# alex-petrenko/sample-factory

Hardware: NVIDIA H100
Metric: env-steps/sec (sampler+learner) at 4096 envs (higher is better)
Workload: dtype f32 (3-pass tf32 hi/lo operand split on wgmma, fp32 accumulate)

## Files before the change

### sample_factory_b200/csrc/rollout_fused.cu

```cuda
#include <cuda.h>

#include <cstdlib>

#include "common.cuh"
#include "gemm.h"
#include "heads_tail.cuh"
#include "tc_ptx.cuh"
#include "wgmma_tile.cuh"

namespace sfb {

constexpr int RF_THREADS = 384;
constexpr int RF_HEAD_AP = 9;
constexpr int RF_MAX_DIM = 128;
constexpr int RF_PRODUCER_REGS = 40;
constexpr int RF_CONSUMER_REGS = 232;

__host__ __device__ __forceinline__ bool rf_wide(int H2) { return H2 >= 256; }
__host__ __device__ __forceinline__ int rf_bm(int H2) { return rf_wide(H2) ? 64 : 128; }
__host__ __device__ __forceinline__ int rf_bn(int H2) { return rf_wide(H2) ? 256 : 128; }

template <bool F16>
struct RfSmem {
    static constexpr int STAGES = 2;
    static constexpr int KBK = F16 ? 64 : TBK;
    __host__ __device__ static constexpr int slot(int bm, int bn) { return F16 ? (bm + bn) * 256 : (bm + 3 * bn) * 128; }
    __host__ __device__ static constexpr int a_bytes(int bm) { return bm * KBK * 4; }
    __host__ __device__ static constexpr int b_hi(int bm, int bn) { return F16 ? bm * 256 : (bm + bn) * 128; }
    __host__ __device__ static constexpr int stage_tx(int bm, int bn) { return (bm + bn) * KBK * 4; }
    static constexpr int OFF_PART = STAGES * slot(64, 256) + 64 * 256;
    static constexpr int OFF_B1 = OFF_PART + (F16 ? 256 * kHeadPartPad * 4 : 0);
    static constexpr int OFF_B2 = OFF_B1 + (F16 ? 256 * 4 : 0);
    static constexpr int OFF_HW = OFF_B2 + (F16 ? 256 * 4 : 0);
    static constexpr int OFF_HB = OFF_HW + (F16 ? RF_HEAD_AP * 256 * 4 : 0);
    static constexpr int OFF_BARS = OFF_HB + (F16 ? 16 * 4 : 0);
    static constexpr int OFF_CSTAT = OFF_BARS + 64;
    static constexpr int TOTAL = OFF_CSTAT + 2 * RF_MAX_DIM * 4 + 1024 ;
    static_assert(2 * STAGES * 8 <= 64 && TOTAL + 64 <= 227 * 1024, "shared memory");
    static_assert(STAGES * slot(128, 128) + 128 * 256 <= OFF_PART, "the 128 x 128 layout fits below the partials");
};


struct RolloutArgs {
    int64_t N; int T, K1, H1, H2;
    const float* b1; const float* b2; const float* wv; const float* wa; int A; const float* bv; const float* ba;
    float* h1; float* part; float* x_norm;
    float* values; int64_t values_rs; float* logits; int64_t logits_rs; float* actions; int64_t actions_rs;
    int32_t* env_actions; float* log_prob; int64_t lp_rs; float* pv_out; int64_t pv_rs; const float* pv_scalar;
    const float* noise; uint64_t seed; int64_t* sampler_step;
    const float* tape; int64_t tape_len; int64_t env_off; int term_period, trunc_period; int64_t* env_step;
    float* env_obs; float* env_rew; uint8_t* env_term; uint8_t* env_trunc;
    float reward_scale, reward_clip; int32_t policy_id; float* t_rew; uint8_t* t_done; uint8_t* t_to; int32_t* t_pid; int64_t stride;
    float* ep_ret; int32_t* ep_len; float* ep_min; float* ep_max; int32_t len_inc; double* stats; float* fin_ret; int32_t* fin_len;
    float* traj_obs; int64_t traj_obs_rs; const float* rnn; int rnn_dim; float* traj_rnn; int64_t traj_rnn_rs;
    const double* mean; const double* var; float sub, inv_scale; int do_sub, do_scale; float eps, clip;
    unsigned int* ticket;
    unsigned long long* trace;
    const float* bound_x; const float* bound_h1;
};

__device__ __forceinline__ void cluster_arrive() { asm volatile("barrier.cluster.arrive.release.aligned;" ::: "memory"); }
__device__ __forceinline__ void cluster_wait() { asm volatile("barrier.cluster.wait.acquire.aligned;" ::: "memory"); }
__device__ __forceinline__ void cluster_sync_all() {
    cluster_arrive();
    cluster_wait();
}
__device__ __forceinline__ void fence_proxy_async_all() { asm volatile("fence.proxy.async.global;" ::: "memory"); }
__device__ __forceinline__ unsigned long long rf_now() {
    unsigned long long t;
    asm volatile("mov.u64 %0, %%globaltimer;" : "=l"(t));
    return t;
}
__device__ __forceinline__ uint32_t smid() {
    uint32_t r;
    asm volatile("mov.u32 %0, %%smid;" : "=r"(r));
    return r;
}
__device__ __forceinline__ uint32_t mapa_shared(uint32_t addr, uint32_t rank) {
    uint32_t r;
    asm volatile("mapa.shared::cluster.u32 %0, %1, %2;" : "=r"(r) : "r"(addr), "r"(rank));
    return r;
}
__device__ __forceinline__ void st_cluster_f4(uint32_t addr, float4 v) {
    asm volatile("st.shared::cluster.v4.f32 [%0], {%1, %2, %3, %4};" ::"r"(addr), "f"(v.x), "f"(v.y), "f"(v.z), "f"(v.w)
                 : "memory");
}
__device__ __forceinline__ uint32_t cluster_ctarank() {
    uint32_t r;
    asm volatile("mov.u32 %0, %%cluster_ctarank;" : "=r"(r));
    return r;
}

template <bool F16>
__device__ __forceinline__ void rf_produce(const CUtensorMap* tmap_x, const CUtensorMap* tmap_w1, const CUtensorMap* tmap_h1,
                                           const CUtensorMap* tmap_w2, int T, int K1, int H1, int bm, int bn, int m0, int n0,
                                           uint8_t* smem, uint64_t* full, uint64_t* empty, bool leader) {
    using S = RfSmem<F16>;
    constexpr int KBK = S::KBK;
    const int slot_bytes = S::slot(bm, bn), b_off = S::a_bytes(bm);
    const uint32_t stage_tx = (uint32_t)S::stage_tx(bm, bn);
    const int n1 = K1 / KBK, n2 = H1 / KBK;
    uint32_t pu = 0;
    auto weight = [&](const CUtensorMap* tb, int kb) {
        const uint32_t s = pu % S::STAGES;
        mbar_wait(&empty[s], ((pu / S::STAGES) & 1) ^ 1);
        mbar_expect_tx(&full[s], stage_tx);
        uint8_t* dst = smem + s * slot_bytes + b_off;
        if (F16) tma_load_3d(dst, tb, &full[s], 64 * kb, n0, 0);
        else tma_load_2d(dst, tb, &full[s], TBK * kb, n0);
        ++pu;
    };
    auto activation = [&](uint32_t u, const CUtensorMap* ta, bool planes, int kb) {
        const uint32_t s = u % S::STAGES;
        if (planes) tma_load_3d(smem + s * slot_bytes, ta, &full[s], 64 * kb, m0, 0);
        else tma_load_2d(smem + s * slot_bytes, ta, &full[s], KBK * kb, m0);
    };
    const int pre2 = n2 < S::STAGES ? n2 : S::STAGES;
    int pre1 = 0;
    for (int t = 0; t < T; ++t) {
        if (leader) {
            fence_proxy_async_all();
            const uint32_t u1 = pu - pre1;
            for (int j = 0; j < n1; ++j) {
                if (j >= pre1) weight(tmap_w1, j);
                activation(u1 + j, tmap_x, false, j);
            }
        }
        __syncwarp();
        cluster_arrive();
        const uint32_t u2 = pu;
        if (leader)
            for (int j = 0; j < pre2; ++j) weight(tmap_w2, j);
        __syncwarp();
        cluster_wait();
        if (leader) {
            fence_proxy_async_all();
            for (int j = 0; j < n2; ++j) {
                if (j >= pre2) weight(tmap_w2, j);
                activation(u2 + j, tmap_h1, F16, j);
            }
        }
        __syncwarp();
        cluster_arrive();
        pre1 = t + 1 < T ? (n1 < S::STAGES ? n1 : S::STAGES) : 0;
        if (leader)
            for (int j = 0; j < pre1; ++j) weight(tmap_w1, j);
        __syncwarp();
        cluster_wait();
        cluster_sync_all();
    }
}

template <bool F16, bool SPLIT_A>
__device__ __forceinline__ void rf_tile(int nkb, bool wide, uint8_t* smem, uint64_t* full, uint64_t* empty, uint32_t& cu,
                                        float (&acc)[64], float (&cross)[64], int ct, int a_shift, unsigned long long* tr,
                                        int s_land, int s_split, int s_done) {
    using S = RfSmem<F16>;
    const int wg = ct >> 7, lt = ct & 127;
    const int bm = wide ? 64 : 128, bn = wide ? 256 : 128;
    const int slot_bytes = S::slot(bm, bn), b_hi = S::b_hi(bm, bn);
    const int a_row = wide ? 0 : 64 * wg, b_row = wide ? 128 * wg : 0;
    uint8_t* conv = smem + S::STAGES * slot_bytes;
#pragma unroll
    for (int i = 0; i < 64; ++i) acc[i] = cross[i] = 0.f;
    int held = -1;
    for (int kb = 0; kb < nkb; ++kb, ++cu) {
        const int s = (int)(cu % S::STAGES);
        uint8_t* slot = smem + s * slot_bytes;
        mbar_wait(&full[s], (cu / S::STAGES) & 1);
        if (tr && kb == nkb - 1) tr[s_land] = rf_now();
        const uint8_t* at = slot;
        if (SPLIT_A || !F16) {
            if (held >= 0) {
                wgmma_wait_all();
                mbar_arrive(&empty[held]);
                held = -1;
                if (wide) consumer_sync();
            }
            if constexpr (F16) {
                if (wide) split_tile_f16<false, 64, 256>(slot, conv, conv + 8192, ct, pow2f_int(a_shift));
                else split_tile_f16<false, 64>(slot + wg * 64 * 256, conv + wg * 8192, conv + 16384 + wg * 8192, lt,
                                               pow2f_int(a_shift));
            } else if (wide) {
                split_tile<false, true, 64, 256>(slot, conv, conv + 8192, ct);
                split_tile<false, true, 256, 256>(slot + 8192, slot + b_hi, slot + b_hi + 32768, ct);
            } else {
                split_tile<false, true, 64>(slot + wg * 64 * 128, conv + wg * 8192, conv + 16384 + wg * 8192, lt);
                split_tile<false, true>(slot + 16384, slot + b_hi, slot + b_hi + 16384, ct);
            }
            fence_proxy_async_smem();
            consumer_sync();
            if (tr && kb == nkb - 1) tr[s_split] = rf_now();
            at = conv;
        }
        const uint64_t da_hi = make_smem_desc(smem_u32(at + a_row * 128));
        const uint64_t da_lo = make_smem_desc(smem_u32(at + bm * 128 + a_row * 128));
        const uint64_t db_hi = make_smem_desc(smem_u32(slot + b_hi + b_row * 128));
        const uint64_t db_lo = make_smem_desc(smem_u32(slot + b_hi + bn * 128 + b_row * 128));
        wgmma_fence();
#pragma unroll
        for (int k = 0; k < TBK / WG_K; ++k) {
            const uint64_t o = (uint64_t)(2 * k);
            if constexpr (F16) {
                wgmma_m64n128k16_f16(acc, da_hi + o, db_hi + o, (kb | k) != 0);
                wgmma_m64n128k16_f16(cross, da_hi + o, db_lo + o, (kb | k) != 0);
                wgmma_m64n128k16_f16(cross, da_lo + o, db_hi + o, 1);
            } else {
                wgmma_m64n128k8_tf32(acc, da_hi + o, db_hi + o, (kb | k) != 0);
                wgmma_m64n128k8_tf32(cross, da_hi + o, db_lo + o, (kb | k) != 0);
                wgmma_m64n128k8_tf32(cross, da_lo + o, db_hi + o, 1);
            }
        }
        wgmma_commit();
        if (held >= 0) {
            wgmma_wait_1();
            mbar_arrive(&empty[held]);
        }
        held = s;
    }
    wgmma_wait_all();
    if (tr) tr[s_done] = rf_now();
    mbar_arrive(&empty[held]);
    if (F16) {
        const float out_scale = pow2f_int(-(a_shift + kF16WShift));
#pragma unroll
        for (int i = 0; i < 64; ++i) acc[i] = fmaf(cross[i], 1.f / 2048.f, acc[i]) * out_scale;
    } else {
#pragma unroll
        for (int i = 0; i < 64; ++i) acc[i] += cross[i];
    }
}

__device__ __forceinline__ void store_h1_split(const float (&acc)[64], int n0, int64_t row_base, int lane, uint16_t* hi,
                                               int64_t lo_off, int64_t M, int H1, const float* bias, int act, float scale) {
    float b[32];
    const float* bp = bias + 2 * (lane & 3);
#pragma unroll
    for (int c = 0; c < 16; ++c) {
        b[2 * c] = bp[8 * c];
        b[2 * c + 1] = bp[8 * c + 1];
    }
#pragma unroll
    for (int j = 0; j < 32; ++j) {
        const int64_t m = row_base + 8 * (j & 1);
        const int n = n0 + 8 * (j >> 1) + 2 * (lane & 3);
        if (m >= M) continue;
        const float v0 = act_fwd_fast(acc[2 * j] + b[j & ~1], act);
        const float v1 = act_fwd_fast(acc[2 * j + 1] + b[j | 1], act);
        uint32_t h, l;
        f16_split2(v0 * scale, v1 * scale, h, l);
        uint16_t* dst = hi + m * H1 + n;
        *reinterpret_cast<uint32_t*>(dst) = h;
        *reinterpret_cast<uint32_t*>(dst + lo_off) = l;
    }
}

template <int ACT>
__device__ __forceinline__ void rf_heads_tile(float (&acc)[64], int nl, int p0, int rb, int lane, const float* b2,
                                              const float* hw, int A, uint32_t part, int rpc) {
    constexpr int JP = 16;
    const int nq = nl + 2 * (lane & 3);
    float b[32];
#pragma unroll
    for (int c = 0; c < 16; ++c) {
        b[2 * c] = b2[nq + 8 * c];
        b[2 * c + 1] = b2[nq + 8 * c + 1];
    }
#pragma unroll
    for (int j = 0; j < 32; ++j) {
        acc[2 * j] = act_fwd_ct<ACT>(acc[2 * j] + b[j & ~1]);
        acc[2 * j + 1] = act_fwd_ct<ACT>(acc[2 * j + 1] + b[j | 1]);
    }
#pragma unroll
    for (int half = 0; half < 2; ++half) {
        float hp[2][kHeadAP];
#pragma unroll
        for (int a = 0; a < kHeadAP; ++a) {
            float s[2] = {0.f, 0.f};
            if (a <= A) {
                const float* w = hw + a * 256 + nq + 64 * half;
                float2 wv[JP / 2];
#pragma unroll
                for (int jj = 0; jj < JP / 2; ++jj) wv[jj] = *reinterpret_cast<const float2*>(w + 8 * jj);
#pragma unroll
                for (int jj = 0; jj < JP / 2; ++jj) {
#pragma unroll
                    for (int rs = 0; rs < 2; ++rs) {
                        const int j = JP * half + 2 * jj + rs;
                        s[rs] = fmaf(acc[2 * j], wv[jj].x, s[rs]);
                        s[rs] = fmaf(acc[2 * j + 1], wv[jj].y, s[rs]);
                    }
                }
            }
#pragma unroll
            for (int rs = 0; rs < 2; ++rs) {
                s[rs] += __shfl_xor_sync(0xffffffffu, s[rs], 1);
                s[rs] += __shfl_xor_sync(0xffffffffu, s[rs], 2);
                hp[rs][a] = s[rs];
            }
        }
        if ((lane & 3) == 0) {
#pragma unroll
            for (int rs = 0; rs < 2; ++rs) {
                const int r = rb + 8 * rs;
                const uint32_t dst =
                    mapa_shared(part + (uint32_t)(((p0 + half) * rpc + r % rpc) * kHeadPartPad * 4), (uint32_t)(r / rpc));
                st_cluster_f4(dst, make_float4(hp[rs][0], hp[rs][1], hp[rs][2], hp[rs][3]));
                st_cluster_f4(dst + 16, make_float4(hp[rs][4], hp[rs][5], hp[rs][6], hp[rs][7]));
                st_cluster_f4(dst + 32, make_float4(hp[rs][8], 0.f, 0.f, 0.f));
            }
        }
    }
}

template <int ACT, bool F16>
__global__ void __launch_bounds__(RF_THREADS, 1)
rollout_mlp2_tape_kernel(const __grid_constant__ CUtensorMap tmap_x, const __grid_constant__ CUtensorMap tmap_w1,
                         const __grid_constant__ CUtensorMap tmap_h1, const __grid_constant__ CUtensorMap tmap_w2,
                         const RolloutArgs a) {
    using S = RfSmem<F16>;
    constexpr int KBK = S::KBK;
    extern __shared__ uint8_t smem_raw[];
    uint8_t* smem = smem_align_1024(smem_raw);
    uint64_t* full = reinterpret_cast<uint64_t*>(smem + S::OFF_BARS);
    uint64_t* empty = full + S::STAGES;
    float* cstat = reinterpret_cast<float*>(smem + S::OFF_CSTAT);
    float* s_part = reinterpret_cast<float*>(smem + S::OFF_PART);
    float* s_b1 = reinterpret_cast<float*>(smem + S::OFF_B1);
    float* s_b2 = reinterpret_cast<float*>(smem + S::OFF_B2);
    float* s_hw = reinterpret_cast<float*>(smem + S::OFF_HW);
    float* s_hb = reinterpret_cast<float*>(smem + S::OFF_HB);

    __shared__ double s_stats[5];
    const int warp = threadIdx.x >> 5, lane = threadIdx.x & 31;
    if (threadIdx.x < 5) s_stats[threadIdx.x] = 0.0;
    const int cx = (int)cluster_ctarank();
    const int CX = gridDim.x;
    const bool wide = rf_wide(a.H2);
    const int BM = rf_bm(a.H2), BN = rf_bn(a.H2);
    const int n0 = cx * BN;
    const int64_t m0 = (int64_t)blockIdx.y * BM;
    const int P = a.H2 / 64;
    const bool do_rms = a.mean != nullptr;
    unsigned long long* cta_trace =
        a.trace ? a.trace + (int64_t)a.T * 16 + 4 * ((int64_t)blockIdx.y * gridDim.x + blockIdx.x) : nullptr;
    if (cta_trace && threadIdx.x == 0) {
        cta_trace[0] = smid();
        cta_trace[1] = rf_now();
    }

    if (threadIdx.x == 0) {
        asm volatile("prefetch.tensormap [%0];" ::"l"(&tmap_x) : "memory");
        asm volatile("prefetch.tensormap [%0];" ::"l"(&tmap_w1) : "memory");
        asm volatile("prefetch.tensormap [%0];" ::"l"(&tmap_h1) : "memory");
        asm volatile("prefetch.tensormap [%0];" ::"l"(&tmap_w2) : "memory");
        for (int s = 0; s < S::STAGES; ++s) {
            mbar_init(&full[s], 1);
            mbar_init(&empty[s], 256);
        }
        fence_barrier_init();
    }
    __syncthreads();
    pdl_wait();
    pdl_trigger();
    if (cta_trace && threadIdx.x == 0) cta_trace[2] = rf_now();
    if (do_rms)
        for (int c = threadIdx.x; c < a.K1; c += RF_THREADS) col_stats(a.mean, a.var, c, a.eps, cstat[c], cstat[a.K1 + c]);
    if (F16) {
        for (int i = threadIdx.x; i < BN; i += RF_THREADS) {
            s_b1[i] = a.b1[n0 + i];
            s_b2[i] = a.b2[n0 + i];
            s_hw[i] = a.wv[n0 + i];
            for (int r = 0; r < a.A; ++r) s_hw[(r + 1) * 256 + i] = a.wa[(int64_t)r * a.H2 + n0 + i];
        }
        if (threadIdx.x <= a.A) s_hb[threadIdx.x] = threadIdx.x == 0 ? a.bv[0] : a.ba[threadIdx.x - 1];
    }
    __syncthreads();
    const int64_t env_step0 = a.env_step[0];
    const uint64_t philox0 = a.sampler_step ? (uint64_t)*a.sampler_step : 0ull;

    if (warp < 4) {
        setmaxnreg_dec<RF_PRODUCER_REGS>();
        rf_produce<F16>(&tmap_x, &tmap_w1, &tmap_h1, &tmap_w2, a.T, a.K1, a.H1, BM, BN, (int)m0, n0, smem, full, empty,
                        threadIdx.x == 0);
    } else {
        setmaxnreg_inc<RF_CONSUMER_REGS>();
        const float pv = a.pv_scalar ? *a.pv_scalar : 0.f;
        const int shift_x = F16 ? f16_shift_for_bound(a.bound_x[0]) : 0;
        const int shift_h = F16 ? f16_shift_for_bound(a.bound_h1[0]) : 0;
        const bool tracer = a.trace != nullptr && blockIdx.x == 0 && blockIdx.y == 0 && threadIdx.x == 128;
#define RF_TRACE(slot) do { if (tracer) a.trace[(int64_t)t * 16 + (slot)] = rf_now(); } while (0)
        uint32_t cu = 0;
        const TcEpilogue epi_heads{1, ACT, a.b2, nullptr, 0, a.wv, a.wa, a.A, a.part};
        const TcEpilogue epi_h1{1, ACT, a.b1, nullptr, 0};
        const int ct = threadIdx.x - 128;
        const int64_t row_base = m0 + (wide ? 0 : (ct >> 7) * 64) + ((ct >> 5) & 3) * 16 + (lane >> 2);
        TileCoord tc;
        tc.m0 = m0; tc.n0 = n0 + (wide ? (ct >> 7) * 128 : 0); tc.k_begin = 0; tc.num_kb = 0; tc.z = 0;

        for (int t = 0; t < a.T; ++t) {
            RF_TRACE(0);
            unsigned long long* const tr = tracer ? a.trace + (int64_t)t * 16 : nullptr;
            {
                float acc[64], cross[64];
                rf_tile<F16, true>(a.K1 / KBK, wide, smem, full, empty, cu, acc, cross, ct, shift_x, tr, 1, 2, 5);
                if (F16)
                    store_h1_split(acc, tc.n0, row_base, lane, reinterpret_cast<uint16_t*>(a.h1), a.N * a.H1, a.N, a.H1,
                                   s_b1 + (tc.n0 - n0), ACT, pow2f_int(shift_h));
                else
                    store_tile(acc, tc, row_base, lane, a.h1, a.H1, a.N, a.H1, 1, epi_h1);
                RF_TRACE(6);
                fence_proxy_async_all();
                RF_TRACE(3);
            }
            cluster_sync_all();
            RF_TRACE(4);
            {
                float acc[64], cross[64];
                rf_tile<F16, !F16>(a.H1 / KBK, wide, smem, full, empty, cu, acc, cross, ct, shift_h, tr, 11, 14, 12);
                if (F16)
                    rf_heads_tile<ACT>(acc, tc.n0 - n0, tc.n0 / 64, (int)(row_base - m0), lane, s_b2, s_hw, a.A,
                                       smem_u32(s_part), BM / CX);
                else
                    heads_tile<ACT>(acc, tc, row_base, lane, nullptr, 0, a.N, a.H2, epi_heads);
                RF_TRACE(7);
            }
            cluster_sync_all();
            RF_TRACE(8);

            {
                const int g = lane & 7;
                const int grp = lane >> 3;
                const int act_idx = (g + 7) & 7;
                const bool has_logit = act_idx < a.A;
                const bool leader = g == 0;
                const bool last = (t + 1 == a.T);
                const int64_t step = env_step0 + t;
                const uint64_t offset = philox0 + (uint64_t)t;
                const float* src_step = a.tape + ((step + 1) % a.tape_len) * a.N * a.K1;
                const float* noise_t = a.noise ? a.noise + (int64_t)t * a.N * a.A : nullptr;
                const int rpc = BM / CX;
                const unsigned gmask = 0xffu << (grp * 8);
                for (int base = 0; base < rpc; base += 32) {
                    const int rr = base + (warp - 4) * 4 + grp;
                    const int64_t row = m0 + cx * rpc + rr;
                    const bool ok = rr < rpc && row < a.N;
                    float x = 0.f, val = 0.f;
                    float ob[RF_MAX_DIM / 8];
                    float er0 = 0.f, mn0 = 0.f, mx0 = 0.f;
                    int32_t el0 = 0;
                    const int cpl = a.K1 >> 3;
                    if (ok) {
                        if (F16) {
                            if (has_logit)
                                for (int p = 0; p < P; ++p) x += s_part[(p * rpc + rr) * kHeadPartPad + 1 + act_idx];
                            if (leader)
                                for (int p = 0; p < P; ++p) val += s_part[(p * rpc + rr) * kHeadPartPad];
                        } else {
                            if (has_logit)
                                for (int p = 0; p < P; ++p) x += a.part[((int64_t)p * a.N + row) * kHeadPartPad + 1 + act_idx];
                            if (leader)
                                for (int p = 0; p < P; ++p) val += a.part[((int64_t)p * a.N + row) * kHeadPartPad];
                        }
                        const float4* src4 = reinterpret_cast<const float4*>(src_step + row * a.K1 + g * cpl);
#pragma unroll
                        for (int q = 0; q < RF_MAX_DIM / 32; ++q)
                            if (4 * q < cpl) {
                                const float4 f4 = src4[q];
                                ob[4 * q] = f4.x; ob[4 * q + 1] = f4.y; ob[4 * q + 2] = f4.z; ob[4 * q + 3] = f4.w;
                            }
                        if (leader && a.ep_ret) { er0 = a.ep_ret[row]; el0 = a.ep_len[row]; mn0 = a.ep_min[row]; mx0 = a.ep_max[row]; }
                    }
                    if (tr && base == 0) tr[13] = tc_now_after(val);
                    x += has_logit ? (F16 ? s_hb[1 + act_idx] : a.ba[act_idx]) : 0.f;
                    val += F16 ? s_hb[0] : a.bv[0];
                    const float xl = has_logit ? x : -INFINITY;
                    float m = xl;
#pragma unroll
                    for (int o = 4; o > 0; o >>= 1) m = fmaxf(m, __shfl_xor_sync(0xffffffffu, m, o));
                    const float ex = has_logit ? expf(xl - m) : 0.f;
                    float ssum = ex;
#pragma unroll
                    for (int o = 4; o > 0; o >>= 1) ssum += __shfl_xor_sync(0xffffffffu, ssum, o);
                    const float pr = __fdiv_rn(ex, ssum);
                    const float logp = (xl - m) - logf(ssum);
                    float q = 1.f;
                    if (ok && has_logit) {
                        if (noise_t) q = noise_t[row * a.A + act_idx];
                        else {
                            curandStatePhilox4_32_10_t st;
                            curand_init(a.seed, (unsigned long long)(row * a.A + act_idx), offset, &st);
                            q = fmaxf(-logf(curand_uniform(&st)), 1.0e-30f);
                        }
                    }
                    float best = has_logit ? __fdiv_rn(pr, q) : -INFINITY;
                    int idx = has_logit ? act_idx : 0x7fffffff;
#pragma unroll
                    for (int o = 4; o > 0; o >>= 1) {
                        const float ob_ = __shfl_xor_sync(0xffffffffu, best, o);
                        const int oi = __shfl_xor_sync(0xffffffffu, idx, o);
                        if (ob_ > best || (ob_ == best && oi < idx)) { best = ob_; idx = oi; }
                    }
                    const float lp = __shfl_sync(0xffffffffu, logp, (grp << 3) | ((idx + 1) & 7));
                    if (tr && base == 0) tr[15] = tc_now_after(lp);
                    (void)gmask;
                    if (!ok) continue;
                    if (has_logit) a.logits[row * a.logits_rs + (int64_t)t * a.A + act_idx] = x;
                    const int64_t env = a.env_off + row;
                    const float r_raw = (float)idx / (float)a.A;
                    const bool tm = ((step * 7 + env * 13) % a.term_period) == 0;
                    const bool tr = (((step + env) % a.trunc_period) == 0) && !tm;
                    float* obs_next = a.traj_obs + row * a.traj_obs_rs + (int64_t)(t + 1) * a.K1 + g * cpl;
                    float* env_o = a.env_obs + row * a.K1 + g * cpl;
                    float* xn = a.x_norm + row * a.K1 + g * cpl;
#pragma unroll
                    for (int q4 = 0; q4 < RF_MAX_DIM / 32; ++q4)
                        if (4 * q4 < cpl) {
                            const float4 f4 = make_float4(ob[4 * q4], ob[4 * q4 + 1], ob[4 * q4 + 2], ob[4 * q4 + 3]);
                            reinterpret_cast<float4*>(env_o)[q4] = f4;
                            reinterpret_cast<float4*>(obs_next)[q4] = f4;
                            if (!last) {
                                const int c = g * cpl + 4 * q4;
                                float4 y;
                                y.x = norm_one(f4.x, a.sub, a.inv_scale, a.do_sub, a.do_scale, do_rms, do_rms ? cstat[c] : 0.f, do_rms ? cstat[a.K1 + c] : 1.f, a.clip);
                                y.y = norm_one(f4.y, a.sub, a.inv_scale, a.do_sub, a.do_scale, do_rms, do_rms ? cstat[c + 1] : 0.f, do_rms ? cstat[a.K1 + c + 1] : 1.f, a.clip);
                                y.z = norm_one(f4.z, a.sub, a.inv_scale, a.do_sub, a.do_scale, do_rms, do_rms ? cstat[c + 2] : 0.f, do_rms ? cstat[a.K1 + c + 2] : 1.f, a.clip);
                                y.w = norm_one(f4.w, a.sub, a.inv_scale, a.do_sub, a.do_scale, do_rms, do_rms ? cstat[c + 3] : 0.f, do_rms ? cstat[a.K1 + c + 3] : 1.f, a.clip);
                                reinterpret_cast<float4*>(xn)[q4] = y;
                            }
                        }
                    if (a.rnn)
                        for (int j = g; j < a.rnn_dim; j += 8)
                            a.traj_rnn[row * a.traj_rnn_rs + (int64_t)(t + 1) * a.rnn_dim + j] = a.rnn[row * a.rnn_dim + j];
                    if (leader) {
                        a.values[row * a.values_rs + t] = val;
                        a.actions[row * a.actions_rs + t] = (float)idx;
                        a.env_actions[row] = idx;
                        a.log_prob[row * a.lp_rs + t] = lp;
                        a.pv_out[row * a.pv_rs + t] = pv;
                        a.env_rew[row] = r_raw;
                        a.env_term[row] = tm;
                        a.env_trunc[row] = tr;
                        const bool done = tm || tr;
                        float r = __fmul_rn(r_raw, a.reward_scale);
                        r = clampf(r, -a.reward_clip, a.reward_clip);
                        a.t_rew[row * a.stride + t] = r;
                        a.t_done[row * a.stride + t] = done ? 1 : 0;
                        a.t_to[row * a.stride + t] = tr ? 1 : 0;
                        a.t_pid[row * a.stride + t] = a.policy_id;
                        if (a.ep_ret) {
                            float er = er0 + r_raw;
                            int32_t el = el0 + a.len_inc;
                            float mn = fminf(mn0, r_raw), mx = fmaxf(mx0, r_raw);
                            if (a.fin_ret) {
                                a.fin_ret[row * a.stride + t] = done ? er : __int_as_float(0x7fc00000);
                                a.fin_len[row * a.stride + t] = done ? el : -1;
                            }
                            if (done) {
                                if (a.stats) {
                                    atomicAdd(&s_stats[0], 1.0); atomicAdd(&s_stats[1], (double)er); atomicAdd(&s_stats[2], (double)el);
                                    atomicAdd(&s_stats[3], (double)mn); atomicAdd(&s_stats[4], (double)mx);
                                }
                                er = 0.f; el = 0; mn = INFINITY; mx = -INFINITY;
                            }
                            a.ep_ret[row] = er; a.ep_len[row] = el; a.ep_min[row] = mn; a.ep_max[row] = mx;
                        }
                    }
                }
                fence_proxy_async_all();
                RF_TRACE(9);
            }

            cluster_sync_all();
            RF_TRACE(10);
        }
#undef RF_TRACE
    }

    __syncthreads();
    if (threadIdx.x < 5 && a.stats && s_stats[0] > 0.0) atomicAdd(a.stats + threadIdx.x, s_stats[threadIdx.x]);
    if (threadIdx.x == 0) {
        if (cta_trace) cta_trace[3] = rf_now();
        __threadfence();
        if (atomicAdd(a.ticket, 1u) == gridDim.x * gridDim.y - 1u) {
            *a.ticket = 0u;
            a.env_step[0] = env_step0 + a.T;
            if (a.sampler_step) *a.sampler_step = (int64_t)philox0 + a.T;
        }
    }
}

template <int ACT, bool F16>
static int rollout_launch_config(int64_t N, int H2, cudaStream_t st, cudaLaunchConfig_t& cfg, cudaLaunchAttribute (&attr)[2]) {
    auto kern = rollout_mlp2_tape_kernel<ACT, F16>;
    static bool attr_set = false;
    if (!attr_set) {
        SFB_CUDA_OK(cudaFuncSetAttribute(kern, cudaFuncAttributeMaxDynamicSharedMemorySize, RfSmem<F16>::TOTAL));
        attr_set = true;
    }
    const int CX = H2 / rf_bn(H2);
    cfg = {};
    cfg.gridDim = dim3((unsigned)CX, (unsigned)ceil_div(N, rf_bm(H2)));
    cfg.blockDim = dim3(RF_THREADS);
    cfg.dynamicSmemBytes = RfSmem<F16>::TOTAL;
    cfg.stream = st;
    attr[0].id = cudaLaunchAttributeClusterDimension;
    attr[0].val.clusterDim.x = (unsigned)CX;
    attr[0].val.clusterDim.y = 1;
    attr[0].val.clusterDim.z = 1;
    attr[1].id = cudaLaunchAttributeProgrammaticStreamSerialization;
    attr[1].val.programmaticStreamSerializationAllowed = 1;
    cfg.attrs = attr;
    cfg.numAttrs = pdl_enabled() ? 2 : 1;
    return 0;
}

template <int ACT, bool F16>
static int launch_rollout(const CUtensorMap* tm, const RolloutArgs& a, cudaStream_t st) {
    cudaLaunchConfig_t cfg;
    cudaLaunchAttribute attr[2];
    const int rc = rollout_launch_config<ACT, F16>(a.N, a.H2, st, cfg, attr);
    if (rc) return rc;
    SFB_CUDA_OK(cudaLaunchKernelEx(&cfg, rollout_mlp2_tape_kernel<ACT, F16>, tm[0], tm[1], tm[2], tm[3], a));
    SFB_LAUNCH_OK();
    return 0;
}

template <int ACT, bool F16>
static int rollout_occupancy(int64_t N, int H2, int* needed, int* resident) {
    cudaLaunchConfig_t cfg;
    cudaLaunchAttribute attr[2];
    const int rc = rollout_launch_config<ACT, F16>(N, H2, 0, cfg, attr);
    if (rc) return rc;
    SFB_CUDA_OK(cudaOccupancyMaxActiveClusters(resident, rollout_mlp2_tape_kernel<ACT, F16>, &cfg));
    *needed = (int)(cfg.gridDim.x * cfg.gridDim.y / attr[0].val.clusterDim.x);
    return 0;
}

int tc_rollout_mlp2_supported(const float* W1, const float* W2, int K1, int H1, int H2, int A, int engine) {
    if (engine != SFB200_GEMM_TC_3XTF32 || !tc_init()) return 0;
    if (!(K1 == 32 || K1 == 64 || K1 == 96 || K1 == 128) || H1 != H2 || !(H2 == 128 || H2 == 256 || H2 == 512)) return 0;
    if (A < 1 || A + 1 > RF_HEAD_AP) return 0;
    if ((reinterpret_cast<uintptr_t>(W1) & 15u) || (reinterpret_cast<uintptr_t>(W2) & 15u)) return 0;
    return 2 * (H2 / 128);
}

static bool rollout_f16_enabled() {
    static int v = -1;
    if (v < 0) {
        const char* e = getenv("SFB200_TC_F16");
        v = (e && e[0] == '0') ? 0 : 1;
    }
    return v == 1;
}

#define SFB_RF_LAUNCH(F16v)                                                                  \
    switch (act) {                                                                           \
        case SFB200_ACT_ELU: return launch_rollout<SFB200_ACT_ELU, F16v>(tm, a, st);     \
        case SFB200_ACT_RELU: return launch_rollout<SFB200_ACT_RELU, F16v>(tm, a, st);   \
        case SFB200_ACT_TANH: return launch_rollout<SFB200_ACT_TANH, F16v>(tm, a, st);   \
        default: return launch_rollout<SFB200_ACT_NONE, F16v>(tm, a, st);                \
    }

static int g_rollout_form = -1;

int tc_rollout_mlp2_tape(const float* W1, const float* W2, int act, int engine, const RolloutArgs& a_in, cudaStream_t st) {
    if (!tc_rollout_mlp2_supported(W1, W2, a_in.K1, a_in.H1, a_in.H2, a_in.A, engine)) return SFB_TC_UNSUPPORTED;
    if ((reinterpret_cast<uintptr_t>(a_in.wv) & 7u) || (reinterpret_cast<uintptr_t>(a_in.wa) & 7u)) return SFB_TC_UNSUPPORTED;
    RolloutArgs a = a_in;
    const uint32_t BM = (uint32_t)rf_bm(a.H2), BN = (uint32_t)rf_bn(a.H2);
    if (rollout_f16_enabled() && a.K1 % 64 == 0 && a.H1 % 64 == 0) {
        const F16Twin t1 = f16_twin_lookup(W1, (int64_t)a.H1 * a.K1), t2 = f16_twin_lookup(W2, (int64_t)a.H2 * a.H1);
        const float* bx = operand_bound_lookup(a.x_norm, a.N * a.K1 * (int64_t)sizeof(float));
        const float* bh = operand_bound_lookup(a.h1, a.N * a.H1 * (int64_t)sizeof(float));
        if (t1.hi && t2.hi && bx && bh) {
            if (f16_check_enabled()) {
                int rc = f16_twins_check(W1, t1, a.H1, a.K1, false, st);
                if (!rc) rc = f16_twins_check(W2, t2, a.H2, a.H1, false, st);
                if (rc) return rc;
            }
            a.bound_x = bx;
            a.bound_h1 = bh;
            CUtensorMap tm[4];
            bool ok = make_tmap(&tm[0], a.x_norm, (uint64_t)a.K1, (uint64_t)a.N, (uint64_t)a.K1, 64, BM);
            ok = ok && make_tmap_f16_twins(&tm[1], t1.hi, t1.lo - t1.hi, (uint64_t)a.K1, (uint64_t)a.H1, BN);
            ok = ok && make_tmap_f16_twins(&tm[2], reinterpret_cast<const uint16_t*>(a.h1), a.N * a.H1, (uint64_t)a.H1,
                                           (uint64_t)a.N, BM);
            ok = ok && make_tmap_f16_twins(&tm[3], t2.hi, t2.lo - t2.hi, (uint64_t)a.H1, (uint64_t)a.H2, BN);
            if (ok) {
                g_rollout_form = 1;
                SFB_RF_LAUNCH(true)
            }
        }
    }
    a.bound_x = a.bound_h1 = nullptr;
    CUtensorMap tm[4];
    bool ok = make_tmap(&tm[0], a.x_norm, (uint64_t)a.K1, (uint64_t)a.N, (uint64_t)a.K1, TBK, BM);
    ok = ok && make_tmap(&tm[1], W1, (uint64_t)a.K1, (uint64_t)a.H1, (uint64_t)a.K1, TBK, BN);
    ok = ok && make_tmap(&tm[2], a.h1, (uint64_t)a.H1, (uint64_t)a.N, (uint64_t)a.H1, TBK, BM);
    ok = ok && make_tmap(&tm[3], W2, (uint64_t)a.H1, (uint64_t)a.H2, (uint64_t)a.H1, TBK, BN);
    if (!ok) return SFB_TC_UNSUPPORTED;
    g_rollout_form = 0;
    SFB_RF_LAUNCH(false)
}
#undef SFB_RF_LAUNCH

}

using namespace sfb;

extern "C" {

static unsigned long long* g_rollout_trace = nullptr;
int sfb200_rollout_set_trace(void* trace_dev) {
    g_rollout_trace = (unsigned long long*)trace_dev;
    return 0;
}

int sfb200_rollout_last_form(void) { return g_rollout_form; }

int sfb200_rollout_occupancy(int64_t n_envs, int K1, int H1, int H2, int A, int engine, int act, int* clusters_needed,
                             int* clusters_resident) {
    SFB_CHECK_ARG(n_envs > 0 && clusters_needed && clusters_resident, "rollout_occupancy: bad arguments");
    SFB_CHECK_ARG(tc_rollout_mlp2_supported(nullptr, nullptr, K1, H1, H2, A, engine),
                  "rollout_occupancy: model not covered (K1=%d H1=%d H2=%d A=%d engine=%d)", K1, H1, H2, A, engine);
    if (rollout_f16_enabled() && K1 % 64 == 0 && H1 % 64 == 0) {
        switch (act) {
            case SFB200_ACT_ELU: return rollout_occupancy<SFB200_ACT_ELU, true>(n_envs, H2, clusters_needed, clusters_resident);
            case SFB200_ACT_RELU: return rollout_occupancy<SFB200_ACT_RELU, true>(n_envs, H2, clusters_needed, clusters_resident);
            case SFB200_ACT_TANH: return rollout_occupancy<SFB200_ACT_TANH, true>(n_envs, H2, clusters_needed, clusters_resident);
            default: return rollout_occupancy<SFB200_ACT_NONE, true>(n_envs, H2, clusters_needed, clusters_resident);
        }
    }
    switch (act) {
        case SFB200_ACT_ELU: return rollout_occupancy<SFB200_ACT_ELU, false>(n_envs, H2, clusters_needed, clusters_resident);
        case SFB200_ACT_RELU: return rollout_occupancy<SFB200_ACT_RELU, false>(n_envs, H2, clusters_needed, clusters_resident);
        case SFB200_ACT_TANH: return rollout_occupancy<SFB200_ACT_TANH, false>(n_envs, H2, clusters_needed, clusters_resident);
        default: return rollout_occupancy<SFB200_ACT_NONE, false>(n_envs, H2, clusters_needed, clusters_resident);
    }
}

int sfb200_rollout_mlp2_partials(const float* W1, const float* W2, int K1, int H1, int H2, int A, int engine) {
    return tc_rollout_mlp2_supported(W1, W2, K1, H1, H2, A, engine);
}

int sfb200_rollout_mlp2_tape(int64_t n_envs, int T, int K1, const float* W1, const float* b1, int H1, const float* W2,
                             const float* b2, int H2, int act, int engine, const float* Wv, const float* bv, const float* Wa,
                             const float* ba, int A, float* h1_scratch, float* head_partials, float* x_norm,
                             float* values_0, int64_t values_stride, float* logits_0, int64_t logits_stride,
                             const float* noise, uint64_t philox_seed, int64_t* sampler_step, float* actions_0,
                             int64_t actions_stride, int32_t* env_actions, float* log_prob_0, int64_t log_prob_stride,
                             const float* policy_version_scalar, float* policy_version_0, int64_t pv_stride,
                             const float* tape, int64_t tape_len, int64_t env_index_offset, int term_period, int trunc_period,
                             int64_t* env_step_counter, float* env_obs, float* env_rew, uint8_t* env_terminated,
                             uint8_t* env_truncated, float reward_scale, float reward_clip, int32_t policy_id,
                             float* traj_rewards_0, uint8_t* traj_dones_0, uint8_t* traj_time_outs_0, int32_t* traj_policy_id_0,
                             int64_t traj_stride, float* ep_return, int32_t* ep_len, float* ep_min_raw, float* ep_max_raw,
                             int32_t len_increment, double* stats, float* fin_return_0, int32_t* fin_len_0, float* traj_obs_0,
                             int64_t traj_obs_stride, const float* rnn, int rnn_dim, float* traj_rnn_0, int64_t traj_rnn_stride,
                             const double* mean, const double* var, float sub_mean, float inv_scale, float eps, float clip,
                             void* stream) {
    SFB_CHECK_ARG(n_envs > 0 && T > 0 && W1 && b1 && W2 && b2 && Wv && bv && Wa && ba && h1_scratch && head_partials && x_norm,
                  "rollout_mlp2_tape: bad model arguments");
    SFB_CHECK_ARG(values_0 && logits_0 && actions_0 && env_actions && log_prob_0 && policy_version_0 && policy_version_scalar,
                  "rollout_mlp2_tape: bad heads arguments");
    SFB_CHECK_ARG(tape && tape_len > 0 && term_period > 0 && trunc_period > 0 && env_step_counter && env_obs && env_rew &&
                      env_terminated && env_truncated, "rollout_mlp2_tape: bad env arguments");
    SFB_CHECK_ARG(traj_rewards_0 && traj_dones_0 && traj_time_outs_0 && traj_policy_id_0 && traj_obs_0,
                  "rollout_mlp2_tape: bad trajectory arguments");
    SFB_CHECK_ARG((mean == nullptr) == (var == nullptr), "rollout_mlp2_tape: mean/var must both be set or both NULL");
    SFB_CHECK_ARG(K1 <= RF_MAX_DIM, "rollout_mlp2_tape: observation rows of up to %d floats", RF_MAX_DIM);
    SFB_CHECK_ARG((reinterpret_cast<uintptr_t>(h1_scratch) & 15u) == 0 && (reinterpret_cast<uintptr_t>(x_norm) & 15u) == 0 &&
                      (reinterpret_cast<uintptr_t>(head_partials) & 15u) == 0, "rollout_mlp2_tape: scratch buffers must be 16-byte aligned");
    const bool with_rnn = rnn && traj_rnn_0 && rnn_dim > 0;
    unsigned int* ticket = reinterpret_cast<unsigned int*>(env_step_counter + 1);
    const RolloutArgs a{n_envs, T, K1, H1, H2, b1, b2, Wv, Wa, A, bv, ba, h1_scratch, head_partials, x_norm,
                        values_0, values_stride, logits_0, logits_stride, actions_0, actions_stride, env_actions, log_prob_0,
                        log_prob_stride, policy_version_0, pv_stride, policy_version_scalar, noise, philox_seed, sampler_step,
                        tape, tape_len, env_index_offset, term_period, trunc_period, env_step_counter, env_obs, env_rew,
                        env_terminated, env_truncated, reward_scale, reward_clip, policy_id, traj_rewards_0, traj_dones_0,
                        traj_time_outs_0, traj_policy_id_0, traj_stride, ep_return, ep_len, ep_min_raw, ep_max_raw, len_increment,
                        stats, fin_return_0, fin_len_0, traj_obs_0, traj_obs_stride, with_rnn ? rnn : nullptr, rnn_dim, traj_rnn_0,
                        traj_rnn_stride, mean, var, sub_mean, inv_scale, fabsf(sub_mean) > 1e-8f ? 1 : 0,
                        fabsf(inv_scale - 1.0f) > 1e-8f ? 1 : 0, eps, clip, ticket, g_rollout_trace, nullptr, nullptr};
    const int rc = tc_rollout_mlp2_tape(W1, W2, act, engine, a, (cudaStream_t)stream);
    SFB_CHECK_ARG(rc != SFB_TC_UNSUPPORTED, "rollout_mlp2_tape: model not covered (K1=%d H1=%d H2=%d A=%d engine=%d); "
                  "sfb200_rollout_mlp2_partials() tells when to use the per-step calls", K1, H1, H2, A, engine);
    return rc;
}

}
```

### sample_factory_b200/csrc/tc_ptx.cuh

```cuda
#pragma once
#include <cuda.h>
#include <cudaTypedefs.h>

#include "common.cuh"

namespace sfb {

constexpr int TBM = 128;
constexpr int TBN = 128;
constexpr int TBK = 32;
constexpr int WG_K = 8;

__device__ __forceinline__ uint32_t smem_u32(const void* p) { return (uint32_t)__cvta_generic_to_shared(p); }
__device__ __forceinline__ uint8_t* smem_align_1024(uint8_t* raw) {
    return raw + ((1024u - (smem_u32(raw) & 1023u)) & 1023u);
}

__device__ __forceinline__ void mbar_init(uint64_t* bar, uint32_t count) {
    asm volatile("mbarrier.init.shared::cta.b64 [%0], %1;" ::"r"(smem_u32(bar)), "r"(count));
}
__device__ __forceinline__ void mbar_expect_tx(uint64_t* bar, uint32_t bytes) {
    asm volatile("mbarrier.arrive.expect_tx.shared::cta.b64 _, [%0], %1;" ::"r"(smem_u32(bar)), "r"(bytes) : "memory");
}
__device__ __forceinline__ void mbar_arrive(uint64_t* bar) {
    asm volatile("mbarrier.arrive.shared::cta.b64 _, [%0];" ::"r"(smem_u32(bar)) : "memory");
}
__device__ __forceinline__ void mbar_wait(uint64_t* bar, uint32_t parity) {
    asm volatile(
        "{\n"
        ".reg .pred P1;\n"
        "WAIT_LOOP:\n"
        "mbarrier.try_wait.parity.shared::cta.b64 P1, [%0], %1;\n"
        "@P1 bra.uni WAIT_DONE;\n"
        "bra.uni WAIT_LOOP;\n"
        "WAIT_DONE:\n"
        "}\n" ::"r"(smem_u32(bar)),
        "r"(parity)
        : "memory");
}
__device__ __forceinline__ void fence_barrier_init() { asm volatile("fence.mbarrier_init.release.cluster;" ::: "memory"); }
__device__ __forceinline__ void fence_proxy_async_smem() { asm volatile("fence.proxy.async.shared::cta;" ::: "memory"); }

__device__ __forceinline__ void tma_load_2d(void* smem_dst, const CUtensorMap* tmap, uint64_t* bar, int c0, int c1) {
    asm volatile(
        "cp.async.bulk.tensor.2d.shared::cluster.global.mbarrier::complete_tx::bytes [%0], [%1, {%3, %4}], [%2];" ::"r"(
            smem_u32(smem_dst)),
        "l"(tmap), "r"(smem_u32(bar)), "r"(c0), "r"(c1)
        : "memory");
}

__device__ __forceinline__ void tma_load_3d(void* smem_dst, const CUtensorMap* tmap, uint64_t* bar, int c0, int c1, int c2) {
    asm volatile(
        "cp.async.bulk.tensor.3d.shared::cluster.global.mbarrier::complete_tx::bytes [%0], [%1, {%3, %4, %5}], [%2];" ::"r"(
            smem_u32(smem_dst)),
        "l"(tmap), "r"(smem_u32(bar)), "r"(c0), "r"(c1), "r"(c2)
        : "memory");
}

__device__ __forceinline__ void wgmma_fence() { asm volatile("wgmma.fence.sync.aligned;" ::: "memory"); }
__device__ __forceinline__ void wgmma_commit() { asm volatile("wgmma.commit_group.sync.aligned;" ::: "memory"); }
__device__ __forceinline__ void wgmma_wait_all() { asm volatile("wgmma.wait_group.sync.aligned 0;" ::: "memory"); }
__device__ __forceinline__ void wgmma_wait_1() { asm volatile("wgmma.wait_group.sync.aligned 1;" ::: "memory"); }

constexpr int kTraceWords = 16;
__device__ __forceinline__ unsigned long long tc_now() {
    unsigned long long t;
    asm volatile("mov.u64 %0, %%globaltimer;" : "=l"(t));
    return t;
}
__device__ __forceinline__ unsigned long long tc_now_after(float dep) {
    unsigned long long t;
    asm volatile(
        "{\n"
        ".reg .pred p;\n"
        "setp.num.f32 p, %1, %1;\n"
        "mov.u64 %0, 0;\n"
        "@p mov.u64 %0, %%globaltimer;\n"
        "}\n"
        : "=l"(t)
        : "f"(dep));
    return t;
}
__device__ __forceinline__ uint32_t tc_smid() {
    uint32_t r;
    asm volatile("mov.u32 %0, %%smid;" : "=r"(r));
    return r;
}

template <int REGS>
__device__ __forceinline__ void setmaxnreg_dec() { asm volatile("setmaxnreg.dec.sync.aligned.u32 %0;" ::"n"(REGS)); }
template <int REGS>
__device__ __forceinline__ void setmaxnreg_inc() { asm volatile("setmaxnreg.inc.sync.aligned.u32 %0;" ::"n"(REGS)); }

__device__ __forceinline__ void wgmma_m64n128k8_tf32(float (&d)[64], uint64_t desc_a, uint64_t desc_b, uint32_t scale_d) {
    asm volatile(
        "{\n"
        ".reg .pred p;\n"
        "setp.ne.b32 p, %66, 0;\n"
        "wgmma.mma_async.sync.aligned.m64n128k8.f32.tf32.tf32 "
        "{%0,%1,%2,%3,%4,%5,%6,%7,%8,%9,%10,%11,%12,%13,%14,%15,%16,%17,%18,%19,%20,%21,%22,%23,%24,%25,%26,%27,%28,%29,%30,%31,%32,%33,%34,%35,%36,%37,%38,%39,%40,%41,%42,%43,%44,%45,%46,%47,%48,%49,%50,%51,%52,%53,%54,%55,%56,%57,%58,%59,%60,%61,%62,%63}, "
        "%64, %65, p, 1, 1;\n"
        "}\n"
        : "+f"(d[0]), "+f"(d[1]), "+f"(d[2]), "+f"(d[3]), "+f"(d[4]), "+f"(d[5]), "+f"(d[6]), "+f"(d[7]), "+f"(d[8]), "+f"(d[9]),
          "+f"(d[10]), "+f"(d[11]), "+f"(d[12]), "+f"(d[13]), "+f"(d[14]), "+f"(d[15]), "+f"(d[16]), "+f"(d[17]), "+f"(d[18]),
          "+f"(d[19]), "+f"(d[20]), "+f"(d[21]), "+f"(d[22]), "+f"(d[23]), "+f"(d[24]), "+f"(d[25]), "+f"(d[26]), "+f"(d[27]),
          "+f"(d[28]), "+f"(d[29]), "+f"(d[30]), "+f"(d[31]), "+f"(d[32]), "+f"(d[33]), "+f"(d[34]), "+f"(d[35]), "+f"(d[36]),
          "+f"(d[37]), "+f"(d[38]), "+f"(d[39]), "+f"(d[40]), "+f"(d[41]), "+f"(d[42]), "+f"(d[43]), "+f"(d[44]), "+f"(d[45]),
          "+f"(d[46]), "+f"(d[47]), "+f"(d[48]), "+f"(d[49]), "+f"(d[50]), "+f"(d[51]), "+f"(d[52]), "+f"(d[53]), "+f"(d[54]),
          "+f"(d[55]), "+f"(d[56]), "+f"(d[57]), "+f"(d[58]), "+f"(d[59]), "+f"(d[60]), "+f"(d[61]), "+f"(d[62]), "+f"(d[63])
        : "l"(desc_a), "l"(desc_b), "r"(scale_d));
}

__device__ __forceinline__ void wgmma_m64n128k16_f16(float (&d)[64], uint64_t desc_a, uint64_t desc_b, uint32_t scale_d) {
    asm volatile(
        "{\n"
        ".reg .pred p;\n"
        "setp.ne.b32 p, %66, 0;\n"
        "wgmma.mma_async.sync.aligned.m64n128k16.f32.f16.f16 "
        "{%0,%1,%2,%3,%4,%5,%6,%7,%8,%9,%10,%11,%12,%13,%14,%15,%16,%17,%18,%19,%20,%21,%22,%23,%24,%25,%26,%27,%28,%29,%30,%31,%32,%33,%34,%35,%36,%37,%38,%39,%40,%41,%42,%43,%44,%45,%46,%47,%48,%49,%50,%51,%52,%53,%54,%55,%56,%57,%58,%59,%60,%61,%62,%63}, "
        "%64, %65, p, 1, 1, 0, 0;\n"
        "}\n"
        : "+f"(d[0]), "+f"(d[1]), "+f"(d[2]), "+f"(d[3]), "+f"(d[4]), "+f"(d[5]), "+f"(d[6]), "+f"(d[7]), "+f"(d[8]),
          "+f"(d[9]), "+f"(d[10]), "+f"(d[11]), "+f"(d[12]), "+f"(d[13]), "+f"(d[14]), "+f"(d[15]), "+f"(d[16]), "+f"(d[17]),
          "+f"(d[18]), "+f"(d[19]), "+f"(d[20]), "+f"(d[21]), "+f"(d[22]), "+f"(d[23]), "+f"(d[24]), "+f"(d[25]), "+f"(d[26]),
          "+f"(d[27]), "+f"(d[28]), "+f"(d[29]), "+f"(d[30]), "+f"(d[31]), "+f"(d[32]), "+f"(d[33]), "+f"(d[34]), "+f"(d[35]),
          "+f"(d[36]), "+f"(d[37]), "+f"(d[38]), "+f"(d[39]), "+f"(d[40]), "+f"(d[41]), "+f"(d[42]), "+f"(d[43]), "+f"(d[44]),
          "+f"(d[45]), "+f"(d[46]), "+f"(d[47]), "+f"(d[48]), "+f"(d[49]), "+f"(d[50]), "+f"(d[51]), "+f"(d[52]), "+f"(d[53]),
          "+f"(d[54]), "+f"(d[55]), "+f"(d[56]), "+f"(d[57]), "+f"(d[58]), "+f"(d[59]), "+f"(d[60]), "+f"(d[61]), "+f"(d[62]),
          "+f"(d[63])
        : "l"(desc_a), "l"(desc_b), "r"(scale_d));
}

template <int TRANS_B>
__device__ __forceinline__ void wgmma_m64n128k16_f16_rs(float (&d)[64], const uint32_t (&a)[4], uint64_t desc_b) {
    asm volatile(
        "{\n"
        ".reg .pred p;\n"
        "setp.ne.b32 p, %70, 0;\n"
        "wgmma.mma_async.sync.aligned.m64n128k16.f32.f16.f16 "
        "{%0,%1,%2,%3,%4,%5,%6,%7,%8,%9,%10,%11,%12,%13,%14,%15,%16,%17,%18,%19,%20,%21,%22,%23,%24,%25,%26,%27,%28,%29,%30,%31,%32,%33,%34,%35,%36,%37,%38,%39,%40,%41,%42,%43,%44,%45,%46,%47,%48,%49,%50,%51,%52,%53,%54,%55,%56,%57,%58,%59,%60,%61,%62,%63}, "
        "{%64, %65, %66, %67}, %68, p, 1, 1, %69;\n"
        "}\n"
        : "+f"(d[0]), "+f"(d[1]), "+f"(d[2]), "+f"(d[3]), "+f"(d[4]), "+f"(d[5]), "+f"(d[6]), "+f"(d[7]), "+f"(d[8]),
          "+f"(d[9]), "+f"(d[10]), "+f"(d[11]), "+f"(d[12]), "+f"(d[13]), "+f"(d[14]), "+f"(d[15]), "+f"(d[16]), "+f"(d[17]),
          "+f"(d[18]), "+f"(d[19]), "+f"(d[20]), "+f"(d[21]), "+f"(d[22]), "+f"(d[23]), "+f"(d[24]), "+f"(d[25]), "+f"(d[26]),
          "+f"(d[27]), "+f"(d[28]), "+f"(d[29]), "+f"(d[30]), "+f"(d[31]), "+f"(d[32]), "+f"(d[33]), "+f"(d[34]), "+f"(d[35]),
          "+f"(d[36]), "+f"(d[37]), "+f"(d[38]), "+f"(d[39]), "+f"(d[40]), "+f"(d[41]), "+f"(d[42]), "+f"(d[43]), "+f"(d[44]),
          "+f"(d[45]), "+f"(d[46]), "+f"(d[47]), "+f"(d[48]), "+f"(d[49]), "+f"(d[50]), "+f"(d[51]), "+f"(d[52]), "+f"(d[53]),
          "+f"(d[54]), "+f"(d[55]), "+f"(d[56]), "+f"(d[57]), "+f"(d[58]), "+f"(d[59]), "+f"(d[60]), "+f"(d[61]), "+f"(d[62]),
          "+f"(d[63])
        : "r"(a[0]), "r"(a[1]), "r"(a[2]), "r"(a[3]), "l"(desc_b), "n"(TRANS_B), "r"(1u));
}

__device__ __forceinline__ uint64_t make_smem_desc(uint32_t smem_addr) {
    uint64_t d = 0;
    d |= (uint64_t)((smem_addr >> 4) & 0x3fff);
    d |= (uint64_t)1 << 16;
    d |= (uint64_t)(1024u >> 4) << 32;
    d |= (uint64_t)1 << 62;
    return d;
}
__device__ __forceinline__ uint64_t make_smem_desc_mn(uint32_t smem_addr) {
    uint64_t d = 0;
    d |= (uint64_t)((smem_addr >> 4) & 0x3fff);
    d |= (uint64_t)(4096u >> 4) << 16;
    d |= (uint64_t)(1024u >> 4) << 32;
    d |= (uint64_t)1 << 62;
    return d;
}
__device__ __forceinline__ uint32_t sw128_offset(int row, int k) {
    return (uint32_t)(row * 128 + ((((k >> 2) ^ row) & 7) << 4) + (k & 3) * 4);
}

template <int ACT>
__device__ __forceinline__ float act_fwd_ct(float z) {
    if (ACT == SFB200_ACT_ELU) {
        float e;
        asm("ex2.approx.ftz.f32 %0, %1;" : "=f"(e) : "f"(z * 1.4426950216293334961f));
        return z > 0.f ? z : e - 1.f;
    }
    if (ACT == SFB200_ACT_RELU) return fmaxf(z, 0.f);
    if (ACT == SFB200_ACT_TANH) return tanhf(z);
    return z;
}
template <int ACT>
__device__ __forceinline__ float act_bwd_ct(float h) {
    if (ACT == SFB200_ACT_ELU) return h > 0.f ? 1.f : h + 1.f;
    if (ACT == SFB200_ACT_RELU) return h > 0.f ? 1.f : 0.f;
    if (ACT == SFB200_ACT_TANH) return 1.f - h * h;
    return 1.f;
}

bool tc_init();
bool make_tmap(CUtensorMap* out, const float* base, uint64_t dim0, uint64_t dim1, uint64_t stride1_elems, uint32_t box0,
               uint32_t box1, bool swizzle128 = false);
bool make_tmap_f16_twins(CUtensorMap* out, const uint16_t* hi, int64_t lo_offset, uint64_t K, uint64_t rows,
                         uint32_t box_rows);

}
```

Measured before the change: 35.19 million.

## Stage h1 f16 hi/lo tiles in swizzled smem and write back via TMA store

The first-layer epilogue no longer scatters 32-bit f16 hi/lo pairs straight to global memory. Each consumer writes them into 128B-swizzled shared-memory boxes, reusing the pipeline slots or conversion buffer, then one thread per group issues a 3D TMA bulk store and waits for it before the cluster sync. This aims to replace many uncoalesced global stores with bulk tensor transfers. It adds consumer barriers, a larger shared-memory layout, and wider per-k-block trace slots.

```diff
diff --git a/sample_factory_b200/csrc/rollout_fused.cu b/sample_factory_b200/csrc/rollout_fused.cu
--- a/sample_factory_b200/csrc/rollout_fused.cu
+++ b/sample_factory_b200/csrc/rollout_fused.cu
@@ -13,6 +13,7 @@
 constexpr int RF_THREADS = 384;
 constexpr int RF_HEAD_AP = 9;
 constexpr int RF_MAX_DIM = 128;
+constexpr int RF_TRACE_WORDS = 32;
 constexpr int RF_PRODUCER_REGS = 40;
 constexpr int RF_CONSUMER_REGS = 232;
 
@@ -28,7 +29,8 @@
     __host__ __device__ static constexpr int a_bytes(int bm) { return bm * KBK * 4; }
     __host__ __device__ static constexpr int b_hi(int bm, int bn) { return F16 ? bm * 256 : (bm + bn) * 128; }
     __host__ __device__ static constexpr int stage_tx(int bm, int bn) { return (bm + bn) * KBK * 4; }
-    static constexpr int OFF_PART = STAGES * slot(64, 256) + 64 * 256;
+    static constexpr int OFF_CONV_END = STAGES * slot(64, 256) + 64 * 256;
+    static constexpr int OFF_PART = OFF_CONV_END + (F16 ? 64 * 256 : 0);
     static constexpr int OFF_B1 = OFF_PART + (F16 ? 256 * kHeadPartPad * 4 : 0);
     static constexpr int OFF_B2 = OFF_B1 + (F16 ? 256 * 4 : 0);
     static constexpr int OFF_HW = OFF_B2 + (F16 ? 256 * 4 : 0);
@@ -38,6 +40,8 @@
     static constexpr int TOTAL = OFF_CSTAT + 2 * RF_MAX_DIM * 4 + 1024 ;
     static_assert(2 * STAGES * 8 <= 64 && TOTAL + 64 <= 227 * 1024, "shared memory");
     static_assert(STAGES * slot(128, 128) + 128 * 256 <= OFF_PART, "the 128 x 128 layout fits below the partials");
+    static_assert(a_bytes(64) % 1024 == 0 && slot(64, 256) % 1024 == 0 && OFF_CONV_END % 1024 == 0,
+                  "h1 staging boxes (slot A regions, conversion buffer, the buffer after it) on 1024 B swizzle atoms");
 };
 
 
@@ -154,7 +158,7 @@
 template <bool F16, bool SPLIT_A>
 __device__ __forceinline__ void rf_tile(int nkb, bool wide, uint8_t* smem, uint64_t* full, uint64_t* empty, uint32_t& cu,
                                         float (&acc)[64], float (&cross)[64], int ct, int a_shift, unsigned long long* tr,
-                                        int s_land, int s_split, int s_done) {
+                                        int s_land, int s_split, int s_done, int s_each) {
     using S = RfSmem<F16>;
     const int wg = ct >> 7, lt = ct & 127;
     const int bm = wide ? 64 : 128, bn = wide ? 256 : 128;
@@ -168,7 +172,11 @@
         const int s = (int)(cu % S::STAGES);
         uint8_t* slot = smem + s * slot_bytes;
         mbar_wait(&full[s], (cu / S::STAGES) & 1);
-        if (tr && kb == nkb - 1) tr[s_land] = rf_now();
+        if (tr) {
+            const unsigned long long now = rf_now();
+            if (kb == nkb - 1) tr[s_land] = now;
+            if (s_each >= 0 && kb < 16) tr[s_each + kb] = now;
+        }
         const uint8_t* at = slot;
         if (SPLIT_A || !F16) {
             if (held >= 0) {
@@ -231,8 +239,9 @@
     }
 }
 
-__device__ __forceinline__ void store_h1_split(const float (&acc)[64], int n0, int64_t row_base, int lane, uint16_t* hi,
-                                               int64_t lo_off, int64_t M, int H1, const float* bias, int act, float scale) {
+__device__ __forceinline__ void store_h1_tma(const float (&acc)[64], const CUtensorMap* tmap_h1, int n0, int m0, int rt,
+                                             int lane, uint8_t* const (&box)[2], int plane_bytes, bool issuer,
+                                             const float* bias, int act, float scale) {
     float b[32];
     const float* bp = bias + 2 * (lane & 3);
 #pragma unroll
@@ -241,17 +250,25 @@
         b[2 * c + 1] = bp[8 * c + 1];
     }
 #pragma unroll
-    for (int j = 0; j < 32; ++j) {
-        const int64_t m = row_base + 8 * (j & 1);
-        const int n = n0 + 8 * (j >> 1) + 2 * (lane & 3);
-        if (m >= M) continue;
-        const float v0 = act_fwd_fast(acc[2 * j] + b[j & ~1], act);
-        const float v1 = act_fwd_fast(acc[2 * j + 1] + b[j | 1], act);
-        uint32_t h, l;
-        f16_split2(v0 * scale, v1 * scale, h, l);
-        uint16_t* dst = hi + m * H1 + n;
-        *reinterpret_cast<uint32_t*>(dst) = h;
-        *reinterpret_cast<uint32_t*>(dst + lo_off) = l;
+    for (int h = 0; h < 2; ++h) {
+#pragma unroll
+        for (int jj = 0; jj < 16; ++jj) {
+            const int j = 16 * h + jj;
+            const int r = rt + 8 * (j & 1), c = (j >> 1) & 7;
+            const float v0 = act_fwd_fast(acc[2 * j] + b[j & ~1], act);
+            const float v1 = act_fwd_fast(acc[2 * j + 1] + b[j | 1], act);
+            uint32_t hv, lv;
+            f16_split2(v0 * scale, v1 * scale, hv, lv);
+            uint8_t* dst = box[h] + r * 128 + (((c ^ r) & 7) << 4) + 4 * (lane & 3);
+            *reinterpret_cast<uint32_t*>(dst) = hv;
+            *reinterpret_cast<uint32_t*>(dst + plane_bytes) = lv;
+        }
+        fence_proxy_async_smem();
+        consumer_sync();
+        if (issuer) {
+            tma_store_3d(tmap_h1, box[h], n0 + 64 * h, m0, 0);
+            bulk_commit();
+        }
     }
 }
 
@@ -343,7 +360,7 @@
     const int P = a.H2 / 64;
     const bool do_rms = a.mean != nullptr;
     unsigned long long* cta_trace =
-        a.trace ? a.trace + (int64_t)a.T * 16 + 4 * ((int64_t)blockIdx.y * gridDim.x + blockIdx.x) : nullptr;
+        a.trace ? a.trace + (int64_t)a.T * RF_TRACE_WORDS + 4 * ((int64_t)blockIdx.y * gridDim.x + blockIdx.x) : nullptr;
     if (cta_trace && threadIdx.x == 0) {
         cta_trace[0] = smid();
         cta_trace[1] = rf_now();
@@ -389,7 +406,7 @@
         const int shift_x = F16 ? f16_shift_for_bound(a.bound_x[0]) : 0;
         const int shift_h = F16 ? f16_shift_for_bound(a.bound_h1[0]) : 0;
         const bool tracer = a.trace != nullptr && blockIdx.x == 0 && blockIdx.y == 0 && threadIdx.x == 128;
-#define RF_TRACE(slot) do { if (tracer) a.trace[(int64_t)t * 16 + (slot)] = rf_now(); } while (0)
+#define RF_TRACE(slot) do { if (tracer) a.trace[(int64_t)t * RF_TRACE_WORDS + (slot)] = rf_now(); } while (0)
         uint32_t cu = 0;
         const TcEpilogue epi_heads{1, ACT, a.b2, nullptr, 0, a.wv, a.wa, a.A, a.part};
         const TcEpilogue epi_h1{1, ACT, a.b1, nullptr, 0};
@@ -398,26 +415,34 @@
         TileCoord tc;
         tc.m0 = m0; tc.n0 = n0 + (wide ? (ct >> 7) * 128 : 0); tc.k_begin = 0; tc.num_kb = 0; tc.z = 0;
 
+        uint8_t* const conv = smem + S::STAGES * S::slot(BM, BN);
+        uint8_t* const h1_box[2] = {wide && ct < 128 ? conv + BM * 256 : smem,
+                                    wide && ct < 128 ? conv : smem + S::slot(BM, BN)};
+        const bool h1_issuer = wide ? (ct & 127) == 0 : ct == 0;
+
         for (int t = 0; t < a.T; ++t) {
             RF_TRACE(0);
-            unsigned long long* const tr = tracer ? a.trace + (int64_t)t * 16 : nullptr;
+            unsigned long long* const tr = tracer ? a.trace + (int64_t)t * RF_TRACE_WORDS : nullptr;
             {
                 float acc[64], cross[64];
-                rf_tile<F16, true>(a.K1 / KBK, wide, smem, full, empty, cu, acc, cross, ct, shift_x, tr, 1, 2, 5);
-                if (F16)
-                    store_h1_split(acc, tc.n0, row_base, lane, reinterpret_cast<uint16_t*>(a.h1), a.N * a.H1, a.N, a.H1,
-                                   s_b1 + (tc.n0 - n0), ACT, pow2f_int(shift_h));
-                else
+                rf_tile<F16, true>(a.K1 / KBK, wide, smem, full, empty, cu, acc, cross, ct, shift_x, tr, 1, 2, 5, -1);
+                if (F16) {
+                    store_h1_tma(acc, &tmap_h1, tc.n0, (int)m0, (int)(row_base - m0), lane, h1_box, BM * 128, h1_issuer,
+                                 s_b1 + (tc.n0 - n0), ACT, pow2f_int(shift_h));
+                    RF_TRACE(6);
+                    if (h1_issuer) bulk_wait_all();
+                } else {
                     store_tile(acc, tc, row_base, lane, a.h1, a.H1, a.N, a.H1, 1, epi_h1);
-                RF_TRACE(6);
-                fence_proxy_async_all();
+                    RF_TRACE(6);
+                    fence_proxy_async_all();
+                }
                 RF_TRACE(3);
             }
             cluster_sync_all();
             RF_TRACE(4);
             {
                 float acc[64], cross[64];
-                rf_tile<F16, !F16>(a.H1 / KBK, wide, smem, full, empty, cu, acc, cross, ct, shift_h, tr, 11, 14, 12);
+                rf_tile<F16, !F16>(a.H1 / KBK, wide, smem, full, empty, cu, acc, cross, ct, shift_h, tr, 11, 14, 12, 16);
                 if (F16)
                     rf_heads_tile<ACT>(acc, tc.n0 - n0, tc.n0 / 64, (int)(row_base - m0), lane, s_b2, s_hw, a.A,
                                        smem_u32(s_part), BM / CX);
diff --git a/sample_factory_b200/csrc/tc_ptx.cuh b/sample_factory_b200/csrc/tc_ptx.cuh
--- a/sample_factory_b200/csrc/tc_ptx.cuh
+++ b/sample_factory_b200/csrc/tc_ptx.cuh
@@ -56,6 +56,14 @@
         "l"(tmap), "r"(smem_u32(bar)), "r"(c0), "r"(c1), "r"(c2)
         : "memory");
 }
+
+__device__ __forceinline__ void tma_store_3d(const CUtensorMap* tmap, const void* smem_src, int c0, int c1, int c2) {
+    asm volatile("cp.async.bulk.tensor.3d.global.shared::cta.bulk_group [%0, {%2, %3, %4}], [%1];" ::"l"(tmap),
+                 "r"(smem_u32(smem_src)), "r"(c0), "r"(c1), "r"(c2)
+                 : "memory");
+}
+__device__ __forceinline__ void bulk_commit() { asm volatile("cp.async.bulk.commit_group;" ::: "memory"); }
+__device__ __forceinline__ void bulk_wait_all() { asm volatile("cp.async.bulk.wait_group 0;" ::: "memory"); }
 
 __device__ __forceinline__ void wgmma_fence() { asm volatile("wgmma.fence.sync.aligned;" ::: "memory"); }
 __device__ __forceinline__ void wgmma_commit() { asm volatile("wgmma.commit_group.sync.aligned;" ::: "memory"); }
```

Measured after the change: 36.39 million (median of 6 runs). 1.03x the previous value.
